# vrgamegirl19/comfyui-vrgamedevgirl

Hardware: NVIDIA H100
Metric: megapixels/sec (grain+LUT+colormatch+sharpen chain) at 4K (higher is better)
Workload: dtype f32

## Files before the change

comfyui-vrgamedevgirl_b200/csrc/vrgdg_kernels.cuh:

```cuda
#pragma once
#include <cuda.h>
#include <cuda_runtime.h>
#include <cuda_fp16.h>
#include <cuda_bf16.h>
#include <stdint.h>
#include "vrgdg_math.cuh"

namespace vrgdg {

enum {
  ST_GRAIN = 1, ST_CM = 2, ST_LUT = 4,
  ST_POST = 8,
  ST_CMF = 16,
  ST_PRE = ST_GRAIN | ST_CM | ST_LUT | ST_CMF
};

template <typename T> struct Elem;
template <> struct Elem<float> {
  static __device__ __forceinline__ float ld(float v) { return v; }
  static __device__ __forceinline__ float st(float v) { return v; }
};
template <> struct Elem<__half> {
  static __device__ __forceinline__ float ld(__half v) { return __half2float(v); }
  static __device__ __forceinline__ __half st(float v) { return __float2half_rn(v); }
};
template <> struct Elem<__nv_bfloat16> {
  static __device__ __forceinline__ float ld(__nv_bfloat16 v) { return __bfloat162float(v); }
  static __device__ __forceinline__ __nv_bfloat16 st(float v) { return __float2bfloat16_rn(v); }
};

template <> struct Elem<uint8_t> {
  static __device__ __forceinline__ float ld(uint8_t v) {
    const float r = 1.0f / 255.0f, f = (float)v, q = __fmul_rn(f, r);
    return __fmaf_rn(__fmaf_rn(-255.0f, q, f), r, q);
  }
  static __device__ __forceinline__ uint8_t st(float v) { return (uint8_t)fminf(fmaxf(mulx(v, 255.0f), 0.0f), 255.0f); }
};

template <typename T> struct Io {
  static constexpr bool BGR = false;
  typedef T noise_t;
  typedef uint4 word_t;
};
template <> struct Io<uint8_t> {
  static constexpr bool BGR = true;
  typedef float noise_t;
  typedef uint32_t word_t;
};
template <typename T> __device__ __forceinline__ float noise_ld(T v) { return Elem<T>::ld(v); }
template <> __device__ __forceinline__ float noise_ld<float>(float v) { return v; }

struct PointParams {
  int B, H, W;
  int64_t hw;
  float gI, gs, goms;
  uint64_t seed;
  int64_t frame0;
  int seed_mode;
  GrainKey gkey;
  const void* ext_noise;
  const float* cm_params;
  float cm_t, cm_omt;
  LutParams lut;
};

#ifndef VRGDG_LUT_POLY
#define VRGDG_LUT_POLY 1
#endif

template <int MASK, bool EXACT>
__device__ __forceinline__ void process_pixel(const PointParams& P, const CmFold& cmf, float zr, float zg, float zb,
                                              float& r, float& g, float& b) {
  if (MASK & ST_GRAIN) {
    if (EXACT) grain_blend_exact(r, g, b, zr, zg, zb, P.gI, P.gs, P.goms);
    else grain_blend_fast(r, g, b, zr, zg, zb, P.gI, P.gs, P.goms);
  }
  if (MASK & ST_CM) {
    colormatch_fold_pixel(r, g, b, cmf);
  }
  if (MASK & ST_CMF) {
    colormatch_from_f(r, g, b, cmf);
  }
  if (MASK & ST_LUT) {
    float x0 = r, x1 = g, x2 = b;
    if (EXACT || !VRGDG_LUT_POLY) lut3d_eval<EXACT>(P.lut, r, g, b);
    else lutp_eval(P.lut, r, g, b);
    if (P.lut.blend < 1.0f) {
      r = lut_blend<EXACT>(x0, r, P.lut.blend, P.lut.one_minus_blend);
      g = lut_blend<EXACT>(x1, g, P.lut.blend, P.lut.one_minus_blend);
      b = lut_blend<EXACT>(x2, b, P.lut.blend, P.lut.one_minus_blend);
    }
  }
}

template <int MASK, bool EXACT>
__device__ __forceinline__ void process_pair(const PointParams& P, const CmFold& cmf, const float* z, float* p) {
  process_pixel<(MASK & ~ST_LUT), EXACT>(P, cmf, z[0], z[1], z[2], p[0], p[1], p[2]);
  process_pixel<(MASK & ~ST_LUT), EXACT>(P, cmf, z[3], z[4], z[5], p[3], p[4], p[5]);
  if (MASK & ST_LUT) {
    float x[6] = {p[0], p[1], p[2], p[3], p[4], p[5]};
    if (EXACT || !VRGDG_LUT_POLY) lut3d_eval2<EXACT>(P.lut, p, p + 3);
    else lutp_eval2(P.lut, p, p + 3);
    if (P.lut.blend < 1.0f) {
#pragma unroll
      for (int i = 0; i < 6; ++i) p[i] = lut_blend<EXACT>(x[i], p[i], P.lut.blend, P.lut.one_minus_blend);
    }
  }
}

template <typename T, int MASK, bool EXACT, bool VEC>
__global__ void __launch_bounds__(256)
k_point(const T* __restrict__ in, T* __restrict__ out, PointParams P,
        int blocks_per_frame, int64_t total_vblocks) {
  typedef typename Io<T>::word_t word_t;
  typedef typename Io<T>::noise_t noise_t;
  constexpr bool BGR = Io<T>::BGR;
  constexpr int PX = VEC ? (int)(3 * sizeof(word_t) / (3 * sizeof(T))) : 1;
  constexpr int NE = PX * 3;
  constexpr bool GRAIN = (MASK & ST_GRAIN) != 0;
  const bool has_ext = GRAIN && (P.ext_noise != nullptr);
  for (int64_t vb = blockIdx.x; vb < total_vblocks; vb += gridDim.x) {
    const int frame = (int)(vb / blocks_per_frame);
    const int bif = (int)(vb - (int64_t)frame * blocks_per_frame);
    const int64_t pix0 = ((int64_t)bif * 256 + threadIdx.x) * PX;
    if (pix0 >= P.hw) continue;
    const int64_t e0 = ((int64_t)frame * P.hw + pix0) * 3;
    const GrainFrame gf = grain_frame(P.seed, P.frame0, frame, P.seed_mode);
    CmFold cmf = {};
    if (MASK & (ST_CM | ST_CMF)) cmf = cm_fold(P.cm_params + (int64_t)frame * 12, P.cm_t, P.cm_omt);
    const uint32_t y = GRAIN ? (uint32_t)pix0 / (uint32_t)P.W : 0u;
    const uint32_t x = GRAIN ? (uint32_t)pix0 - y * (uint32_t)P.W : 0u;

    float v[NE];
    float nz[NE];
    union { word_t q[3]; T e[NE]; } u;
    if (VEC) {
      const word_t* src = reinterpret_cast<const word_t*>(in + e0);
      u.q[0] = __ldg(src); u.q[1] = __ldg(src + 1); u.q[2] = __ldg(src + 2);
    } else {
#pragma unroll
      for (int i = 0; i < NE; ++i) u.e[i] = in[e0 + i];
    }
#pragma unroll
    for (int j = 0; j < PX; ++j) {
#pragma unroll
      for (int c = 0; c < 3; ++c) v[3 * j + c] = Elem<T>::ld(u.e[3 * j + (BGR ? 2 - c : c)]);
    }
    if (has_ext) {
      const noise_t* ns = reinterpret_cast<const noise_t*>(P.ext_noise) + e0;
      if (VEC && sizeof(noise_t) == sizeof(T)) {
        union { word_t q[3]; noise_t e[NE]; } n;
        const word_t* nq = reinterpret_cast<const word_t*>(ns);
        n.q[0] = __ldg(nq); n.q[1] = __ldg(nq + 1); n.q[2] = __ldg(nq + 2);
#pragma unroll
        for (int i = 0; i < NE; ++i) nz[i] = noise_ld<noise_t>(n.e[i]);
      } else {
#pragma unroll
        for (int i = 0; i < NE; ++i) nz[i] = noise_ld<noise_t>(ns[i]);
      }
    }
    if (VEC) {
#pragma unroll
      for (int j = 0; j < PX; j += 2) {
        float z[6] = {0.f, 0.f, 0.f, 0.f, 0.f, 0.f};
        if (GRAIN) {
          if (has_ext) {
#pragma unroll
            for (int i = 0; i < 6; ++i) z[i] = nz[3 * j + i];
          } else {
            grain_pair_normals(grain_pair_bits(P.gkey, gf, (x >> 1) + (uint32_t)(j >> 1), y), z);
          }
        }
        process_pair<MASK, EXACT>(P, cmf, z, &v[3 * j]);
      }
    } else {
      float zr = 0.f, zg = 0.f, zb = 0.f;
      if (GRAIN) {
        if (has_ext) { zr = nz[0]; zg = nz[1]; zb = nz[2]; }
        else grain_pixel_normals(P.gkey, gf, x, y, zr, zg, zb);
      }
      process_pixel<MASK, EXACT>(P, cmf, zr, zg, zb, v[0], v[1], v[2]);
    }
#pragma unroll
    for (int j = 0; j < PX; ++j) {
#pragma unroll
      for (int c = 0; c < 3; ++c) u.e[3 * j + (BGR ? 2 - c : c)] = Elem<T>::st(v[3 * j + c]);
    }
    if (VEC) {
      word_t* dst = reinterpret_cast<word_t*>(out + e0);
      dst[0] = u.q[0]; dst[1] = u.q[1]; dst[2] = u.q[2];
// ... 383 lines not shown
  uint8_t* base = smem_raw + (((smem_a + 127u) & ~127u) - smem_a);
  T* stage0 = reinterpret_cast<T*>(base);
  constexpr bool GPLANE = C::GPLANE;
  float* work = reinterpret_cast<float*>(base + (size_t)NS * C::STAGE_BYTES);
  float* gplane = reinterpret_cast<float*>(base + (size_t)NS * C::STAGE_BYTES + (WORK ? ROWS * BX * 4 : 0));
  uint64_t* bars = reinterpret_cast<uint64_t*>(base + (size_t)NS * C::STAGE_BYTES + (WORK ? ROWS * BX * 4 : 0) + (GPLANE ? ROWS * BX * 4 : 0));

  const int tid = threadIdx.x;
  const uint32_t first = blockIdx.x, stride = gridDim.x, total = (uint32_t)Q.total_tiles;
  const uint32_t n_my = (total > first) ? (total - first + stride - 1) / stride : 0;
  const uint32_t tiles_per_frame = (uint32_t)(Q.tiles_x * Q.tiles_y);
  const bool tma = Q.use_tma != 0;

  if (tma && tid == 0) {
#pragma unroll
    for (int s = 0; s < NS; ++s) mbar_init(&bars[s], 1);
    fence_mbar_init();
    fence_proxy_async();
  }
  __syncthreads();

  auto tile_coords = [&](uint32_t k, int& frame, int& y0, int& x0e) {
    const uint32_t t = first + k * stride;
    const uint32_t f = t / tiles_per_frame;
    const uint32_t rem = t - f * tiles_per_frame;
    const uint32_t ty = rem / (uint32_t)Q.tiles_x;
    frame = (int)f;
    y0 = (int)ty * TY;
    x0e = (int)(rem - ty * (uint32_t)Q.tiles_x) * TXE;
  };
  auto issue = [&](uint32_t k) {
    int frame, y0, x0e;
    tile_coords(k, frame, y0, x0e);
    int s = (int)(k % NS);
    mbar_arrive_expect_tx(&bars[s], (uint32_t)C::STAGE_BYTES);
    tma_load_3d(reinterpret_cast<uint8_t*>(stage0) + (size_t)s * C::STAGE_BYTES, &tmap, x0e - PADL, y0 - 1, frame, &bars[s]);
  };

#ifndef VRGDG_EARLY_REFILL
#define VRGDG_EARLY_REFILL 1
#endif
  constexpr bool EARLY = WORK && (VRGDG_EARLY_REFILL != 0);
  constexpr bool LATE1 = !EARLY && NS == 1;
  constexpr uint32_t AHEAD = EARLY ? NS : (LATE1 ? 1 : NS - 1);
  if (tma && tid == 0) {
    for (uint32_t k = 0; k < AHEAD && k < n_my; ++k) issue(k);
  }

  for (uint32_t k = 0; k < n_my; ++k) {
    int frame, y0, x0e;
    tile_coords(k, frame, y0, x0e);
    const int s = tma ? (int)(k % NS) : 0;
    T* raw = reinterpret_cast<T*>(reinterpret_cast<uint8_t*>(stage0) + (size_t)s * C::STAGE_BYTES);

    if (tma) {
      if (!EARLY && !LATE1 && tid == 0 && k + NS - 1 < n_my) {
        fence_proxy_async();
        issue(k + NS - 1);
      }
      mbar_wait(&bars[s], (uint32_t)((k / NS) & 1));
    } else {
      const T* fbase = in + (int64_t)frame * Q.H * Q.RW;
      for (int i = tid; i < ROWS * BX; i += NT) {
        int r = i / BX, c = i - r * BX;
        int y = y0 - 1 + r, x = x0e - PADL + c;
        T v = Elem<T>::st(0.0f);
        if (y >= 0 && y < Q.H && x >= 0 && x < Q.RW) v = fbase[(int64_t)y * Q.RW + x];
        raw[i] = v;
      }
      __syncthreads();
    }

    if ((MASK & ST_PRE) != 0 || WORK || GPLANE) {
      const PointParams& P = Q.P;
      constexpr bool GRAIN = (MASK & ST_GRAIN) != 0;
      constexpr bool BGR = Io<T>::BGR;
      typedef typename Io<T>::noise_t noise_t;
      const GrainFrame gf = grain_frame(P.seed, P.frame0, frame, P.seed_mode);
      CmFold cmf = {};
      if (MASK & (ST_CM | ST_CMF)) cmf = cm_fold(P.cm_params + (int64_t)frame * 12, P.cm_t, P.cm_omt);
      const bool has_ext = GRAIN && (P.ext_noise != nullptr);
      const GrainFrame pgf = grain_frame(Q.pseed, Q.pframe0, frame, Q.pseed_mode);
      const int pair0 = x0e / 6 - 1;
      for (int i = tid; i < ROWS * C::PAIRS; i += NT) {
        const int r = i / C::PAIRS, kx = i - r * C::PAIRS;
        const int y = y0 - 1 + r, pair = pair0 + kx;
        const int pxa = pair * 2;
        const int so = r * BX + PADL - 6 + 6 * kx;
        const bool rowin = (y >= 0 && y < Q.H);
        const bool need_a = (kx > 0), need_b = (kx < C::PAIRS - 1);
        const bool in_a = need_a && rowin && pxa >= 0 && pxa < Q.W;
        const bool in_b = need_b && rowin && pxa + 1 >= 0 && pxa + 1 < Q.W;
        if (GPLANE) {
          float gz[6] = {0.f, 0.f, 0.f, 0.f, 0.f, 0.f};
          if (rowin && pair >= 0 && pxa < Q.W) {
            float z[6];
            grain_pair_normals(grain_pair_bits(Q.pkey, pgf, (uint32_t)pair, (uint32_t)y), z);
            const float gy0 = Q.poms * z[1], gy1 = Q.poms * z[4];
            const float r0 = fmaf(2.0f * Q.ps, z[0], gy0), g0 = fmaf(Q.ps, z[1], gy0), b0 = fmaf(3.0f * Q.ps, z[2], gy0);
            const float r1 = fmaf(2.0f * Q.ps, z[3], gy1), g1 = fmaf(Q.ps, z[4], gy1), b1 = fmaf(3.0f * Q.ps, z[5], gy1);
            gz[0] = BGR ? b0 : r0; gz[1] = g0; gz[2] = BGR ? r0 : b0;
            gz[3] = BGR ? b1 : r1; gz[4] = g1; gz[5] = BGR ? r1 : b1;
          }
          pair_store6(gplane + so, kx > 0, gz);
        }
        if ((MASK & ST_PRE) == 0 && !WORK) continue;
        float e[6] = {0.f, 0.f, 0.f, 0.f, 0.f, 0.f};
        if (in_a | in_b) {
          pair_load6<T>(raw + so, kx > 0, e);
          float z[6] = {0.f, 0.f, 0.f, 0.f, 0.f, 0.f};
          if (GRAIN) {
            if (has_ext) {
              const noise_t* ns = reinterpret_cast<const noise_t*>(P.ext_noise) + ((int64_t)frame * P.hw + (int64_t)y * Q.W + pxa) * 3;
              if (in_a) { z[0] = noise_ld<noise_t>(ns[0]); z[1] = noise_ld<noise_t>(ns[1]); z[2] = noise_ld<noise_t>(ns[2]); }
              if (in_b) { z[3] = noise_ld<noise_t>(ns[3]); z[4] = noise_ld<noise_t>(ns[4]); z[5] = noise_ld<noise_t>(ns[5]); }
            } else {
              grain_pair_normals(grain_pair_bits(P.gkey, gf, (uint32_t)pair, (uint32_t)y), z);
            }
          }
          float p[6] = {e[BGR ? 2 : 0], e[1], e[BGR ? 0 : 2], e[BGR ? 5 : 3], e[4], e[BGR ? 3 : 5]};
          process_pair<MASK, EXACT>(P, cmf, z, p);
          if (in_a) { e[BGR ? 2 : 0] = p[0]; e[1] = p[1]; e[BGR ? 0 : 2] = p[2]; } else if (WORK) { e[0] = 0.f; e[1] = 0.f; e[2] = 0.f; }
          if (in_b) { e[BGR ? 5 : 3] = p[3]; e[4] = p[4]; e[BGR ? 3 : 5] = p[5]; } else if (WORK) { e[3] = 0.f; e[4] = 0.f; e[5] = 0.f; }
        }
        if constexpr (WORK) {
          pair_store6(work + so, kx > 0, e);
        } else {
          if (in_a | in_b) pair_store6(reinterpret_cast<float*>(raw) + so, kx > 0, e);
        }
      }
      __syncthreads();
      if (EARLY && tma && tid == 0 && k + NS < n_my) {
        fence_proxy_async();
        issue(k + NS);
      }
    }

    if (Q.border == 0) {
      if constexpr (WORK) fix_border<float, C>(work, y0, x0e, Q.H, Q.RW);
      else fix_border<T, C>(raw, y0, x0e, Q.H, Q.RW);
    }

    {
      const float* wt = WORK ? work : nullptr;
      if (Q.exact_stencil) {
        switch (Q.op) {
          case 1: stencil_rows<T, 1, MASK, true>(raw, wt, gplane, out, Q, frame, y0, x0e); break;
          case 2: stencil_rows<T, 2, MASK, true>(raw, wt, gplane, out, Q, frame, y0, x0e); break;
          case 3: stencil_rows<T, 3, MASK, false>(raw, wt, gplane, out, Q, frame, y0, x0e); break;
          case 4: stencil_rows<T, 4, MASK, true>(raw, wt, gplane, out, Q, frame, y0, x0e); break;
          case 5: stencil_rows<T, 5, MASK, false>(raw, wt, gplane, out, Q, frame, y0, x0e); break;
          default: stencil_rows<T, 0, MASK, false>(raw, wt, gplane, out, Q, frame, y0, x0e); break;
        }
      } else {
        switch (Q.op) {
          case 1: stencil_rows<T, 1, MASK, false>(raw, wt, gplane, out, Q, frame, y0, x0e); break;
          case 2: stencil_rows<T, 2, MASK, false>(raw, wt, gplane, out, Q, frame, y0, x0e); break;
          case 3: stencil_rows<T, 3, MASK, false>(raw, wt, gplane, out, Q, frame, y0, x0e); break;
          case 4: stencil_rows<T, 4, MASK, false>(raw, wt, gplane, out, Q, frame, y0, x0e); break;
          case 5: stencil_rows<T, 5, MASK, false>(raw, wt, gplane, out, Q, frame, y0, x0e); break;
          default: stencil_rows<T, 0, MASK, false>(raw, wt, gplane, out, Q, frame, y0, x0e); break;
        }
      }
    }
    if (tma) fence_proxy_async();
    __syncthreads();
    if (LATE1 && tma && tid == 0 && k + 1 < n_my) issue(k + 1);
  }
}

constexpr int MOMENT_BLOCKS = 592;
constexpr int MOMENT_UNIT = 128;

__device__ __forceinline__ double warp_sum(double v) {
#pragma unroll
  for (int o = 16; o > 0; o >>= 1) v += __shfl_xor_sync(0xffffffffu, v, o);
  return v;
}

__device__ __forceinline__ void moments_add(float& r, float& g, float& b, float* s1, float* s2) {
  float fx, fy, fz;
  rgb_to_fxyz(r, g, b, fx, fy, fz);
  r = fx; g = fy; b = fz;
  const float u1 = fx - fy, u2 = fy - fz;
  s1[0] += fy; s1[1] += u1; s1[2] += u2;
  s2[0] = fmaf(fy, fy, s2[0]); s2[1] = fmaf(u1, u1, s2[1]); s2[2] = fmaf(u2, u2, s2[2]);
}

#ifndef VRGDG_MOMENT_SMALL_MINB
#define VRGDG_MOMENT_SMALL_MINB 10
#endif
template <int NT> struct MomentLaunch { static constexpr int MINB = (NT == MOMENT_UNIT) ? VRGDG_MOMENT_SMALL_MINB : 4; };
template <typename T, bool GRAIN, bool VEC, int NT>
__global__ void __launch_bounds__(NT, (MomentLaunch<NT>::MINB))
k_lab_moments(const T* __restrict__ in, PointParams P, int row0, int rows, double* __restrict__ partials, float* __restrict__ fplanes) {
  static_assert(NT % MOMENT_UNIT == 0, "whole reduction units per block");
  constexpr int UPB = NT / MOMENT_UNIT;
  const int unit = blockIdx.x * UPB + (threadIdx.x / MOMENT_UNIT), ut = threadIdx.x % MOMENT_UNIT;
  typedef typename Io<T>::word_t word_t;
  typedef typename Io<T>::noise_t noise_t;
  constexpr bool BGR = Io<T>::BGR;
  constexpr int PX = VEC ? (int)(sizeof(word_t) / sizeof(T)) : 1;
  constexpr int NE = PX * 3;
  const int frame = blockIdx.y;
  const int64_t pbeg = (int64_t)row0 * P.W, n = (int64_t)rows * P.W;
  const T* fbase = in + (int64_t)frame * P.hw * 3;
  const GrainFrame gf = grain_frame(P.seed, P.frame0, frame, P.seed_mode);
  const bool has_ext = GRAIN && (P.ext_noise != nullptr);
  const CmFold nocm = {};
// ... 186 lines not shown
```

comfyui-vrgamedevgirl_b200/csrc/vrgdg_math.cuh:

```cuda
#pragma once
#include <stdint.h>
#include <stddef.h>
#include <string.h>
#include <math.h>

#if defined(__CUDACC__)
#define VRGDG_HD __host__ __device__ __forceinline__
#else
#define VRGDG_HD inline
#endif

namespace vrgdg {

#if defined(__CUDA_ARCH__)
VRGDG_HD float addx(float a, float b) { return __fadd_rn(a, b); }
VRGDG_HD float subx(float a, float b) { return __fsub_rn(a, b); }
VRGDG_HD float mulx(float a, float b) { return __fmul_rn(a, b); }
VRGDG_HD float divx(float a, float b) { return __fdiv_rn(a, b); }
VRGDG_HD float sqrtx(float a) { return __fsqrt_rn(a); }
#else
VRGDG_HD float addx(float a, float b) { volatile float r = a + b; return r; }
VRGDG_HD float subx(float a, float b) { volatile float r = a - b; return r; }
VRGDG_HD float mulx(float a, float b) { volatile float r = a * b; return r; }
VRGDG_HD float divx(float a, float b) { volatile float r = a / b; return r; }
// ... 93 lines not shown
#if defined(__CUDA_ARCH__)
  float l2, rr, sn, cs;
  asm("lg2.approx.ftz.f32 %0, %1;" : "=f"(l2) : "f"(u));
  asm("sqrt.approx.ftz.f32 %0, %1;" : "=f"(rr) : "f"(l2 * -1.3862943611198906f));
  asm("sin.approx.ftz.f32 %0, %1;" : "=f"(sn) : "f"(th));
  asm("cos.approx.ftz.f32 %0, %1;" : "=f"(cs) : "f"(th));
#else
  float rr = sqrtf(-2.0f * logf(u));
  float sn = sinf(th), cs = cosf(th);
#endif
  c = rr * cs;
  s = rr * sn;
}

VRGDG_HD void grain_fields(U4 r, uint32_t* rad, uint32_t* ang) {
  const uint32_t M = 0x1FFFFFu;
  rad[0] = r.x & M;
  ang[0] = ((r.x >> 21) | (r.y << 11)) & M;
  rad[1] = (r.y >> 10) & M;
  ang[1] = r.z & M;
  rad[2] = ((r.z >> 21) | (r.w << 11)) & M;
  ang[2] = (r.w >> 10) & M;
}

VRGDG_HD void grain_pair_normals(U4 r, float* z) {
  uint32_t rad[3], ang[3];
  grain_fields(r, rad, ang);
  float c0, s0, c1, s1, c2, s2;
  box_muller21(rad[0], ang[0], c0, s0);
  box_muller21(rad[1], ang[1], c1, s1);
  box_muller21(rad[2], ang[2], c2, s2);
  z[0] = c0; z[1] = s0; z[2] = c1;
  z[3] = s1; z[4] = c2; z[5] = s2;
}

VRGDG_HD void grain_lane_normals(U4 r, int lane, float& zr, float& zg, float& zb) {
  uint32_t rad[3], ang[3];
  grain_fields(r, rad, ang);
  float c1, s1, ca, sa;
  box_muller21(rad[1], ang[1], c1, s1);
  box_muller21(lane ? rad[2] : rad[0], lane ? ang[2] : ang[0], ca, sa);
  zr = lane ? s1 : ca;
  zg = lane ? ca : sa;
  zb = lane ? sa : c1;
}

VRGDG_HD void grain_pixel_normals(const GrainKey& K, const GrainFrame& f, uint32_t x, uint32_t y, float& zr, float& zg, float& zb) {
  grain_lane_normals(grain_pair_bits(K, f, x >> 1, y), (int)(x & 1u), zr, zg, zb);
}

VRGDG_HD void grain_blend_exact(float& r, float& g, float& b, float zr, float zg, float zb,
                                float I, float s, float oms) {
  float zr2 = mulx(zr, 2.0f);
  float zb3 = mulx(zb, 3.0f);
  float gy = mulx(oms, zg);
  float gr = addx(mulx(s, zr2), gy);
  float gg = addx(mulx(s, zg), gy);
  float gb = addx(mulx(s, zb3), gy);
  r = clamp01(addx(r, mulx(gr, I)));
  g = clamp01(addx(g, mulx(gg, I)));
  b = clamp01(addx(b, mulx(gb, I)));
}

VRGDG_HD void grain_blend_fast(float& r, float& g, float& b, float zr, float zg, float zb,
                               float I, float s, float oms) {
  float gy = oms * zg;
  r = clamp01(fmaf(I, fmaf(2.0f * s, zr, gy), r));
  g = clamp01(fmaf(I, fmaf(s, zg, gy), g));
  b = clamp01(fmaf(I, fmaf(3.0f * s, zb, gy), b));
}

struct LutParams {
  const float* lut;
  const float* lutp;
  int S;
  float smax;
  float dmin[3], dspan[3];
  float blend, one_minus_blend;
  int unit_domain;
};

constexpr int LUT_CELL_FLOATS = 24;

struct F8 { float v[8]; };

VRGDG_HD F8 lut_load8(const float* p) {
  F8 q;
#if defined(__CUDA_ARCH__)
  asm("ld.global.nc.v4.f32 {%0,%1,%2,%3}, [%4];"
      : "=f"(q.v[0]), "=f"(q.v[1]), "=f"(q.v[2]), "=f"(q.v[3]) : "l"(p));
  asm("ld.global.nc.v4.f32 {%0,%1,%2,%3}, [%4+16];"
      : "=f"(q.v[4]), "=f"(q.v[5]), "=f"(q.v[6]), "=f"(q.v[7]) : "l"(p));
#else
  for (int i = 0; i < 8; ++i) q.v[i] = p[i];
#endif
  return q;
}

VRGDG_HD void lut_pack_entry(const float* lut3, int S, int b, int g, int r, float* dst24) {
  const int b1 = (b + 1 < S) ? b + 1 : S - 1, g1 = (g + 1 < S) ? g + 1 : S - 1, r1 = (r + 1 < S) ? r + 1 : S - 1;
  const int cb[8] = {b, b, b, b, b1, b1, b1, b1};
  const int cg[8] = {g, g, g1, g1, g, g, g1, g1};
  const int cr[8] = {r, r1, r, r1, r, r1, r, r1};
#pragma unroll
  for (int k = 0; k < 8; ++k) {
    const float* a = lut3 + ((size_t)(cb[k] * S + cg[k]) * S + cr[k]) * 3;
    dst24[k] = a[0]; dst24[8 + k] = a[1]; dst24[16 + k] = a[2];
  }
}

VRGDG_HD void lut_coord(float v, float dmin, float dspan, bool unit, float smax, int S, int& i0, int& i1, float& f) {
  float n = unit ? v : divx(subx(v, dmin), dspan);
  n = clamp01(n);
  float c = mulx(n, smax);
  float fl = floorf(c);
  i0 = (int)fl;
  i1 = (i0 + 1 < S - 1) ? i0 + 1 : S - 1;
  f = subx(c, fl);
}

template <bool EXACT>
VRGDG_HD float lerp_ref(float a, float b, float f, float omf) {
  if (EXACT) return addx(mulx(a, omf), mulx(b, f));
  return fmaf(f, b - a, a);
}

template <bool EXACT>
VRGDG_HD float lut_channel(const F8& q, float fr, float fg, float fb, float omr, float omg, float omb) {
  const float c00 = lerp_ref<EXACT>(q.v[0], q.v[4], fb, omb);
  const float c01 = lerp_ref<EXACT>(q.v[2], q.v[6], fb, omb);
  const float c10 = lerp_ref<EXACT>(q.v[1], q.v[5], fb, omb);
  const float c11 = lerp_ref<EXACT>(q.v[3], q.v[7], fb, omb);
  const float c0 = lerp_ref<EXACT>(c00, c01, fg, omg);
  const float c1 = lerp_ref<EXACT>(c10, c11, fg, omg);
  return clamp01(lerp_ref<EXACT>(c0, c1, fr, omr));
}

template <bool EXACT>
VRGDG_HD void lut3d_eval(const LutParams& P, float& r, float& g, float& b) {
  int r0, r1, g0, g1, b0, b1;
  float fr, fg, fb;
  lut_coord(r, P.dmin[0], P.dspan[0], P.unit_domain != 0, P.smax, P.S, r0, r1, fr);
  lut_coord(g, P.dmin[1], P.dspan[1], P.unit_domain != 0, P.smax, P.S, g0, g1, fg);
  lut_coord(b, P.dmin[2], P.dspan[2], P.unit_domain != 0, P.smax, P.S, b0, b1, fb);
  (void)r1; (void)g1; (void)b1;
  const float* p = P.lut + (size_t)((b0 * P.S + g0) * P.S + r0) * LUT_CELL_FLOATS;
  const F8 q0 = lut_load8(p), q1 = lut_load8(p + 8), q2 = lut_load8(p + 16);
  const float omb = subx(1.0f, fb), omg = subx(1.0f, fg), omr = subx(1.0f, fr);
  r = lut_channel<EXACT>(q0, fr, fg, fb, omr, omg, omb);
  g = lut_channel<EXACT>(q1, fr, fg, fb, omr, omg, omb);
  b = lut_channel<EXACT>(q2, fr, fg, fb, omr, omg, omb);
}

template <bool EXACT>
VRGDG_HD float lut3d_eval_channel(const LutParams& P, float r, float g, float b, int ch) {
  int r0, r1, g0, g1, b0, b1;
  float fr, fg, fb;
  lut_coord(r, P.dmin[0], P.dspan[0], P.unit_domain != 0, P.smax, P.S, r0, r1, fr);
  lut_coord(g, P.dmin[1], P.dspan[1], P.unit_domain != 0, P.smax, P.S, g0, g1, fg);
  lut_coord(b, P.dmin[2], P.dspan[2], P.unit_domain != 0, P.smax, P.S, b0, b1, fb);
  (void)r1; (void)g1; (void)b1;
  const F8 q = lut_load8(P.lut + (size_t)((b0 * P.S + g0) * P.S + r0) * LUT_CELL_FLOATS + 8 * ch);
  return lut_channel<EXACT>(q, fr, fg, fb, subx(1.0f, fr), subx(1.0f, fg), subx(1.0f, fb));
}

struct LutCell { const float* p; float fr, fg, fb; };

VRGDG_HD LutCell lut_locate(const LutParams& P, float r, float g, float b) {
  int r0, r1, g0, g1, b0, b1;
  LutCell c;
  lut_coord(r, P.dmin[0], P.dspan[0], P.unit_domain != 0, P.smax, P.S, r0, r1, c.fr);
  lut_coord(g, P.dmin[1], P.dspan[1], P.unit_domain != 0, P.smax, P.S, g0, g1, c.fg);
  lut_coord(b, P.dmin[2], P.dspan[2], P.unit_domain != 0, P.smax, P.S, b0, b1, c.fb);
  (void)r1; (void)g1; (void)b1;
  c.p = P.lut + (size_t)((b0 * P.S + g0) * P.S + r0) * LUT_CELL_FLOATS;
  return c;
}

template <bool EXACT>
VRGDG_HD void lut_finish(const LutCell& c, const F8& q0, const F8& q1, const F8& q2, float& r, float& g, float& b) {
  const float omb = subx(1.0f, c.fb), omg = subx(1.0f, c.fg), omr = subx(1.0f, c.fr);
  r = lut_channel<EXACT>(q0, c.fr, c.fg, c.fb, omr, omg, omb);
  g = lut_channel<EXACT>(q1, c.fr, c.fg, c.fb, omr, omg, omb);
  b = lut_channel<EXACT>(q2, c.fr, c.fg, c.fb, omr, omg, omb);
}

template <bool EXACT>
VRGDG_HD void lut3d_eval2(const LutParams& P, float* a, float* b) {
  const LutCell ca = lut_locate(P, a[0], a[1], a[2]), cb = lut_locate(P, b[0], b[1], b[2]);
  const F8 a0 = lut_load8(ca.p), a1 = lut_load8(ca.p + 8), a2 = lut_load8(ca.p + 16);
  const F8 b0 = lut_load8(cb.p), b1 = lut_load8(cb.p + 8), b2 = lut_load8(cb.p + 16);
  lut_finish<EXACT>(ca, a0, a1, a2, a[0], a[1], a[2]);
  lut_finish<EXACT>(cb, b0, b1, b2, b[0], b[1], b[2]);
}

VRGDG_HD void lutp_pack_entry(const float* lut3, int S, int b, int g, int r, float* dst24) {
  float c[LUT_CELL_FLOATS];
  lut_pack_entry(lut3, S, b, g, r, c);
#pragma unroll
  for (int ch = 0; ch < 3; ++ch) {
    double k[8];
#pragma unroll
    for (int i = 0; i < 8; ++i) k[i] = (double)c[8 * ch + i];
#pragma unroll
    for (int bit = 1; bit < 8; bit <<= 1) {
#pragma unroll
      for (int i = 0; i < 8; ++i) if (i & bit) k[i] -= k[i ^ bit];
    }
#pragma unroll
    for (int i = 0; i < 8; ++i) dst24[8 * ch + i] = (float)k[i];
  }
}

VRGDG_HD float lutp_channel(const F8& q, float fr, float fg, float fb) {
  const float a0 = fmaf(fb, q.v[4], q.v[0]), b0 = fmaf(fb, q.v[5], q.v[1]);
  const float a1 = fmaf(fb, q.v[6], q.v[2]), b1 = fmaf(fb, q.v[7], q.v[3]);
  return clamp01(fmaf(fr, fmaf(fg, b1, b0), fmaf(fg, a1, a0)));
}

VRGDG_HD LutCell lutp_locate(const LutParams& P, float r, float g, float b) {
  LutCell c = lut_locate(P, r, g, b);
  c.p = P.lutp + (c.p - P.lut);
  return c;
}
VRGDG_HD void lutp_eval(const LutParams& P, float& r, float& g, float& b) {
  const LutCell c = lutp_locate(P, r, g, b);
  const F8 q0 = lut_load8(c.p), q1 = lut_load8(c.p + 8), q2 = lut_load8(c.p + 16);
  r = lutp_channel(q0, c.fr, c.fg, c.fb); g = lutp_channel(q1, c.fr, c.fg, c.fb); b = lutp_channel(q2, c.fr, c.fg, c.fb);
}
VRGDG_HD void lutp_eval2(const LutParams& P, float* a, float* b) {
  const LutCell ca = lutp_locate(P, a[0], a[1], a[2]), cb = lutp_locate(P, b[0], b[1], b[2]);
  const F8 a0 = lut_load8(ca.p), a1 = lut_load8(ca.p + 8), a2 = lut_load8(ca.p + 16);
  const F8 b0 = lut_load8(cb.p), b1 = lut_load8(cb.p + 8), b2 = lut_load8(cb.p + 16);
  a[0] = lutp_channel(a0, ca.fr, ca.fg, ca.fb); a[1] = lutp_channel(a1, ca.fr, ca.fg, ca.fb); a[2] = lutp_channel(a2, ca.fr, ca.fg, ca.fb);
  b[0] = lutp_channel(b0, cb.fr, cb.fg, cb.fb); b[1] = lutp_channel(b1, cb.fr, cb.fg, cb.fb); b[2] = lutp_channel(b2, cb.fr, cb.fg, cb.fb);
}

template <bool EXACT>
VRGDG_HD float lut_blend(float x, float y, float blend, float omb) {
  if (EXACT) return addx(mulx(x, omb), mulx(y, blend));
  return fmaf(y, blend, x * omb);
}

VRGDG_HD float approx_pow(float x, float e) {
#if defined(__CUDA_ARCH__)
  float l, r;
  asm("lg2.approx.ftz.f32 %0, %1;" : "=f"(l) : "f"(x));
  asm("ex2.approx.ftz.f32 %0, %1;" : "=f"(r) : "f"(l * e));
  return r;
#else
  return exp2f(log2f(x) * e) * (1.0f + 3e-7f);
#endif
}
VRGDG_HD float approx_rcp(float x) {
#if defined(__CUDA_ARCH__)
  float r;
  asm("rcp.approx.ftz.f32 %0, %1;" : "=f"(r) : "f"(x));
  return r;
#else
  return 1.0f / x;
#endif
}
VRGDG_HD float cbrt_pos(float x) {
  const float r = approx_pow(x, -0.33333334f);
  const float r3 = (r * r) * r;
  const float rn = r * fmaf(x * r3, -0.33333334f, 1.3333334f);
  return (x * rn) * rn;
}
VRGDG_HD float inv_root5_pos(float x) {
  const float r = approx_pow(x, -0.2f);
  const float r2 = r * r, r4 = r2 * r2;
  return r * fmaf((x * r) * r4, -0.2f, 1.2f);
}
VRGDG_HD float root5_pos(float x) {
  const float r = inv_root5_pos(x);
  const float r2 = r * r;
  return x * (r2 * r2);
}
VRGDG_HD float pow_2p4(float x) {
  const float s = x * inv_root5_pos(x);
  return (s * s) * s;
}
VRGDG_HD float pow_inv2p4(float x) {
  float y = approx_pow(x, 0.083333336f);
  float y2 = y * y, y4 = y2 * y2, y8 = y4 * y4, y11 = (y8 * y2) * y;
  y = fmaf(fmaf(-y11, y, x), approx_rcp(12.0f * y11), y);
  y2 = y * y;
  return (y2 * y2) * y;
}

VRGDG_HD float srgb_to_linear(float c) {
  const float p = pow_2p4(fmaf(fmaxf(c, 0.04045f), (float)(1.0 / 1.055), (float)(0.055 / 1.055)));
  const float l = c * (float)(1.0 / 12.92);
  return (c > 0.04045f) ? p : l;
}
VRGDG_HD float linear_to_srgb(float l) {
  const float p = fmaf(1.055f, approx_pow(fmaxf(l, 0.0031308f), 0.41666666f), -0.055f);
  const float q = 12.92f * l;
  return (l > 0.0031308f) ? p : q;
}
VRGDG_HD float lab_f(float t) {
  const float p = cbrt_pos(fmaxf(t, 0.008856f));
  const float q = fmaf(7.787f, t, (float)(4.0 / 29.0));
  return (t > 0.008856f) ? p : q;
}
VRGDG_HD void rgb_to_fxyz(float r, float g, float b, float& fx, float& fy, float& fz) {
  const float lr = srgb_to_linear(r), lg = srgb_to_linear(g), lb = srgb_to_linear(b);
  const float x = fmaf((float)(0.180423 / 0.95047), lb, fmaf((float)(0.357580 / 0.95047), lg, (float)(0.412453 / 0.95047) * lr));
  const float y = fmaf(0.072169f, lb, fmaf(0.715160f, lg, 0.212671f * lr));
  const float z = fmaf((float)(0.950227 / 1.08883), lb, fmaf((float)(0.119193 / 1.08883), lg, (float)(0.019334 / 1.08883) * lr));
  fx = lab_f(x); fy = lab_f(y); fz = lab_f(z);
}
VRGDG_HD void rgb_to_lab(float r, float g, float b, float& L, float& A, float& Bv) {
  float fx, fy, fz;
  rgb_to_fxyz(r, g, b, fx, fy, fz);
  L = fmaf(116.0f, fy, -16.0f);
  A = 500.0f * (fx - fy);
  Bv = 200.0f * (fy - fz);
}
// ... 110 lines not shown
```

Baseline: 29030.

## Split 3D LUT cell loads across lane pairs with shuffle exchange

Reorders the packed LUT cell layout so each 4-float half holds one r-slice, then has adjacent lanes share LUT lookups: each lane loads only its half of the cell for both its own and its partner's pixels, computes partial trilinear results, and exchanges them via warp shuffles. The stencil tile loop is made warp-uniform so every lane takes part in the shuffles, with per-lane task guards on the stores. The aim is fewer wide scattered loads per lane and better load coalescing across a lane pair, in exchange for extra shuffle instructions and idle lanes running the LUT path on out-of-range tasks.

Result: faster. 32400, median of 6 (+11.6%).

```diff
diff --git a/comfyui-vrgamedevgirl_b200/csrc/vrgdg_kernels.cuh b/comfyui-vrgamedevgirl_b200/csrc/vrgdg_kernels.cuh
--- a/comfyui-vrgamedevgirl_b200/csrc/vrgdg_kernels.cuh
+++ b/comfyui-vrgamedevgirl_b200/csrc/vrgdg_kernels.cuh
@@ -93,19 +93,24 @@
   }
 }
 
+template <bool EXACT, bool LANE_PAIR>
+__device__ __forceinline__ void lut_pair(const PointParams& P, float* p) {
+  constexpr bool POLY = !EXACT && VRGDG_LUT_POLY;
+  float x[6] = {p[0], p[1], p[2], p[3], p[4], p[5]};
+  if (LANE_PAIR) lut_eval_lane_pair<POLY, EXACT>(P.lut, p, p + 3);
+  else if (POLY) lutp_eval2(P.lut, p, p + 3);
+  else lut3d_eval2<EXACT>(P.lut, p, p + 3);
+  if (P.lut.blend < 1.0f) {
+#pragma unroll
+    for (int i = 0; i < 6; ++i) p[i] = lut_blend<EXACT>(x[i], p[i], P.lut.blend, P.lut.one_minus_blend);
+  }
+}
+
 template <int MASK, bool EXACT>
 __device__ __forceinline__ void process_pair(const PointParams& P, const CmFold& cmf, const float* z, float* p) {
   process_pixel<(MASK & ~ST_LUT), EXACT>(P, cmf, z[0], z[1], z[2], p[0], p[1], p[2]);
   process_pixel<(MASK & ~ST_LUT), EXACT>(P, cmf, z[3], z[4], z[5], p[3], p[4], p[5]);
-  if (MASK & ST_LUT) {
-    float x[6] = {p[0], p[1], p[2], p[3], p[4], p[5]};
-    if (EXACT || !VRGDG_LUT_POLY) lut3d_eval2<EXACT>(P.lut, p, p + 3);
-    else lutp_eval2(P.lut, p, p + 3);
-    if (P.lut.blend < 1.0f) {
-#pragma unroll
-      for (int i = 0; i < 6; ++i) p[i] = lut_blend<EXACT>(x[i], p[i], P.lut.blend, P.lut.one_minus_blend);
-    }
-  }
+  if (MASK & ST_LUT) lut_pair<EXACT, false>(P, p);
 }
 
 template <typename T, int MASK, bool EXACT, bool VEC>
@@ -655,12 +660,15 @@
       const bool has_ext = GRAIN && (P.ext_noise != nullptr);
       const GrainFrame pgf = grain_frame(Q.pseed, Q.pframe0, frame, Q.pseed_mode);
       const int pair0 = x0e / 6 - 1;
-      for (int i = tid; i < ROWS * C::PAIRS; i += NT) {
+      constexpr int TASKS = ROWS * C::PAIRS;
+      for (int i0 = tid & ~31; i0 < TASKS; i0 += NT) {
+        const int i = i0 + (tid & 31);
+        const bool task = i < TASKS;
         const int r = i / C::PAIRS, kx = i - r * C::PAIRS;
         const int y = y0 - 1 + r, pair = pair0 + kx;
         const int pxa = pair * 2;
         const int so = r * BX + PADL - 6 + 6 * kx;
-        const bool rowin = (y >= 0 && y < Q.H);
+        const bool rowin = task && (y >= 0 && y < Q.H);
         const bool need_a = (kx > 0), need_b = (kx < C::PAIRS - 1);
         const bool in_a = need_a && rowin && pxa >= 0 && pxa < Q.W;
         const bool in_b = need_b && rowin && pxa + 1 >= 0 && pxa + 1 < Q.W;
@@ -675,10 +683,11 @@
             gz[0] = BGR ? b0 : r0; gz[1] = g0; gz[2] = BGR ? r0 : b0;
             gz[3] = BGR ? b1 : r1; gz[4] = g1; gz[5] = BGR ? r1 : b1;
           }
-          pair_store6(gplane + so, kx > 0, gz);
+          if (task) pair_store6(gplane + so, kx > 0, gz);
         }
         if ((MASK & ST_PRE) == 0 && !WORK) continue;
         float e[6] = {0.f, 0.f, 0.f, 0.f, 0.f, 0.f};
+        float p[6] = {0.f, 0.f, 0.f, 0.f, 0.f, 0.f};
         if (in_a | in_b) {
           pair_load6<T>(raw + so, kx > 0, e);
           float z[6] = {0.f, 0.f, 0.f, 0.f, 0.f, 0.f};
@@ -691,13 +700,16 @@
               grain_pair_normals(grain_pair_bits(P.gkey, gf, (uint32_t)pair, (uint32_t)y), z);
             }
           }
-          float p[6] = {e[BGR ? 2 : 0], e[1], e[BGR ? 0 : 2], e[BGR ? 5 : 3], e[4], e[BGR ? 3 : 5]};
-          process_pair<MASK, EXACT>(P, cmf, z, p);
+          p[0] = e[BGR ? 2 : 0]; p[1] = e[1]; p[2] = e[BGR ? 0 : 2]; p[3] = e[BGR ? 5 : 3]; p[4] = e[4]; p[5] = e[BGR ? 3 : 5];
+          process_pair<(MASK & ~ST_LUT), EXACT>(P, cmf, z, p);
+        }
+        if (MASK & ST_LUT) lut_pair<EXACT, true>(P, p);
+        if (in_a | in_b) {
           if (in_a) { e[BGR ? 2 : 0] = p[0]; e[1] = p[1]; e[BGR ? 0 : 2] = p[2]; } else if (WORK) { e[0] = 0.f; e[1] = 0.f; e[2] = 0.f; }
           if (in_b) { e[BGR ? 5 : 3] = p[3]; e[4] = p[4]; e[BGR ? 3 : 5] = p[5]; } else if (WORK) { e[3] = 0.f; e[4] = 0.f; e[5] = 0.f; }
         }
         if constexpr (WORK) {
-          pair_store6(work + so, kx > 0, e);
+          if (task) pair_store6(work + so, kx > 0, e);
         } else {
           if (in_a | in_b) pair_store6(reinterpret_cast<float*>(raw) + so, kx > 0, e);
         }
diff --git a/comfyui-vrgamedevgirl_b200/csrc/vrgdg_math.cuh b/comfyui-vrgamedevgirl_b200/csrc/vrgdg_math.cuh
--- a/comfyui-vrgamedevgirl_b200/csrc/vrgdg_math.cuh
+++ b/comfyui-vrgamedevgirl_b200/csrc/vrgdg_math.cuh
@@ -199,26 +199,32 @@
 
 constexpr int LUT_CELL_FLOATS = 24;
 
+struct F4 { float v[4]; };
 struct F8 { float v[8]; };
 
-VRGDG_HD F8 lut_load8(const float* p) {
-  F8 q;
+VRGDG_HD F4 lut_load4(const float* p) {
+  F4 q;
 #if defined(__CUDA_ARCH__)
   asm("ld.global.nc.v4.f32 {%0,%1,%2,%3}, [%4];"
       : "=f"(q.v[0]), "=f"(q.v[1]), "=f"(q.v[2]), "=f"(q.v[3]) : "l"(p));
-  asm("ld.global.nc.v4.f32 {%0,%1,%2,%3}, [%4+16];"
-      : "=f"(q.v[4]), "=f"(q.v[5]), "=f"(q.v[6]), "=f"(q.v[7]) : "l"(p));
-#else
-  for (int i = 0; i < 8; ++i) q.v[i] = p[i];
-#endif
+#else
+  for (int i = 0; i < 4; ++i) q.v[i] = p[i];
+#endif
+  return q;
+}
+
+VRGDG_HD F8 lut_load8(const float* p) {
+  const F4 lo = lut_load4(p), hi = lut_load4(p + 4);
+  F8 q;
+  for (int i = 0; i < 4; ++i) { q.v[i] = lo.v[i]; q.v[4 + i] = hi.v[i]; }
   return q;
 }
 
 VRGDG_HD void lut_pack_entry(const float* lut3, int S, int b, int g, int r, float* dst24) {
   const int b1 = (b + 1 < S) ? b + 1 : S - 1, g1 = (g + 1 < S) ? g + 1 : S - 1, r1 = (r + 1 < S) ? r + 1 : S - 1;
-  const int cb[8] = {b, b, b, b, b1, b1, b1, b1};
+  const int cb[8] = {b, b1, b, b1, b, b1, b, b1};
   const int cg[8] = {g, g, g1, g1, g, g, g1, g1};
-  const int cr[8] = {r, r1, r, r1, r, r1, r, r1};
+  const int cr[8] = {r, r, r, r, r1, r1, r1, r1};
 #pragma unroll
   for (int k = 0; k < 8; ++k) {
     const float* a = lut3 + ((size_t)(cb[k] * S + cg[k]) * S + cr[k]) * 3;
@@ -243,14 +249,17 @@
 }
 
 template <bool EXACT>
+VRGDG_HD float lut_half(const float* h, float fg, float fb, float omg, float omb) {
+  const float cx0 = lerp_ref<EXACT>(h[0], h[1], fb, omb);
+  const float cx1 = lerp_ref<EXACT>(h[2], h[3], fb, omb);
+  return lerp_ref<EXACT>(cx0, cx1, fg, omg);
+}
+template <bool EXACT>
+VRGDG_HD float lut_combine(float c0, float c1, float fr, float omr) { return clamp01(lerp_ref<EXACT>(c0, c1, fr, omr)); }
+
+template <bool EXACT>
 VRGDG_HD float lut_channel(const F8& q, float fr, float fg, float fb, float omr, float omg, float omb) {
-  const float c00 = lerp_ref<EXACT>(q.v[0], q.v[4], fb, omb);
-  const float c01 = lerp_ref<EXACT>(q.v[2], q.v[6], fb, omb);
-  const float c10 = lerp_ref<EXACT>(q.v[1], q.v[5], fb, omb);
-  const float c11 = lerp_ref<EXACT>(q.v[3], q.v[7], fb, omb);
-  const float c0 = lerp_ref<EXACT>(c00, c01, fg, omg);
-  const float c1 = lerp_ref<EXACT>(c10, c11, fg, omg);
-  return clamp01(lerp_ref<EXACT>(c0, c1, fr, omr));
+  return lut_combine<EXACT>(lut_half<EXACT>(q.v, fg, fb, omg, omb), lut_half<EXACT>(q.v + 4, fg, fb, omg, omb), fr, omr);
 }
 
 template <bool EXACT>
@@ -283,14 +292,18 @@
 
 struct LutCell { const float* p; float fr, fg, fb; };
 
+VRGDG_HD int lut_cell_offset(const LutParams& P, float r, float g, float b, float& fr, float& fg, float& fb) {
+  int r0, r1, g0, g1, b0, b1;
+  lut_coord(r, P.dmin[0], P.dspan[0], P.unit_domain != 0, P.smax, P.S, r0, r1, fr);
+  lut_coord(g, P.dmin[1], P.dspan[1], P.unit_domain != 0, P.smax, P.S, g0, g1, fg);
+  lut_coord(b, P.dmin[2], P.dspan[2], P.unit_domain != 0, P.smax, P.S, b0, b1, fb);
+  (void)r1; (void)g1; (void)b1;
+  return ((b0 * P.S + g0) * P.S + r0) * LUT_CELL_FLOATS;
+}
+
 VRGDG_HD LutCell lut_locate(const LutParams& P, float r, float g, float b) {
-  int r0, r1, g0, g1, b0, b1;
   LutCell c;
-  lut_coord(r, P.dmin[0], P.dspan[0], P.unit_domain != 0, P.smax, P.S, r0, r1, c.fr);
-  lut_coord(g, P.dmin[1], P.dspan[1], P.unit_domain != 0, P.smax, P.S, g0, g1, c.fg);
-  lut_coord(b, P.dmin[2], P.dspan[2], P.unit_domain != 0, P.smax, P.S, b0, b1, c.fb);
-  (void)r1; (void)g1; (void)b1;
-  c.p = P.lut + (size_t)((b0 * P.S + g0) * P.S + r0) * LUT_CELL_FLOATS;
+  c.p = P.lut + lut_cell_offset(P, r, g, b, c.fr, c.fg, c.fb);
   return c;
 }
 
@@ -320,7 +333,7 @@
 #pragma unroll
     for (int i = 0; i < 8; ++i) k[i] = (double)c[8 * ch + i];
 #pragma unroll
-    for (int bit = 1; bit < 8; bit <<= 1) {
+    for (int bit = 4; bit >= 1; bit >>= 1) {
 #pragma unroll
       for (int i = 0; i < 8; ++i) if (i & bit) k[i] -= k[i ^ bit];
     }
@@ -329,10 +342,11 @@
   }
 }
 
+VRGDG_HD float lutp_half(const float* h, float fg, float fb) { return fmaf(fg, fmaf(fb, h[3], h[2]), fmaf(fb, h[1], h[0])); }
+VRGDG_HD float lutp_combine(float a, float b, float fr) { return clamp01(fmaf(fr, b, a)); }
+
 VRGDG_HD float lutp_channel(const F8& q, float fr, float fg, float fb) {
-  const float a0 = fmaf(fb, q.v[4], q.v[0]), b0 = fmaf(fb, q.v[5], q.v[1]);
-  const float a1 = fmaf(fb, q.v[6], q.v[2]), b1 = fmaf(fb, q.v[7], q.v[3]);
-  return clamp01(fmaf(fr, fmaf(fg, b1, b0), fmaf(fg, a1, a0)));
+  return lutp_combine(lutp_half(q.v, fg, fb), lutp_half(q.v + 4, fg, fb), fr);
 }
 
 VRGDG_HD LutCell lutp_locate(const LutParams& P, float r, float g, float b) {
@@ -352,6 +366,52 @@
   a[0] = lutp_channel(a0, ca.fr, ca.fg, ca.fb); a[1] = lutp_channel(a1, ca.fr, ca.fg, ca.fb); a[2] = lutp_channel(a2, ca.fr, ca.fg, ca.fb);
   b[0] = lutp_channel(b0, cb.fr, cb.fg, cb.fb); b[1] = lutp_channel(b1, cb.fr, cb.fg, cb.fb); b[2] = lutp_channel(b2, cb.fr, cb.fg, cb.fb);
 }
+
+#if defined(__CUDACC__)
+template <bool POLY, bool EXACT>
+__device__ __forceinline__ void lut_eval_lane_pair(const LutParams& P, float* a, float* b) {
+  const unsigned FULL = 0xffffffffu;
+  const bool odd = (threadIdx.x & 1) != 0;
+  float fr[2], fg[2], fb[2];
+  int cell[2];
+  cell[0] = lut_cell_offset(P, a[0], a[1], a[2], fr[0], fg[0], fb[0]);
+  cell[1] = lut_cell_offset(P, b[0], b[1], b[2], fr[1], fg[1], fb[1]);
+  int qc[4];
+  float qg[4], qb[4];
+#pragma unroll
+  for (int k = 0; k < 2; ++k) {
+    const int pc = __shfl_xor_sync(FULL, cell[k], 1);
+    const float pg = __shfl_xor_sync(FULL, fg[k], 1), pb = __shfl_xor_sync(FULL, fb[k], 1);
+    qc[k] = odd ? pc : cell[k];     qg[k] = odd ? pg : fg[k];     qb[k] = odd ? pb : fb[k];
+    qc[2 + k] = odd ? cell[k] : pc; qg[2 + k] = odd ? fg[k] : pg; qb[2 + k] = odd ? fb[k] : pb;
+  }
+  const float* tab = (POLY ? P.lutp : P.lut) + (odd ? 4 : 0);
+  F4 q[4][3];
+#pragma unroll
+  for (int k = 0; k < 4; ++k)
+#pragma unroll
+    for (int ch = 0; ch < 3; ++ch) q[k][ch] = lut_load4(tab + qc[k] + 8 * ch);
+  float h[4][3];
+#pragma unroll
+  for (int k = 0; k < 4; ++k) {
+    const float omg = subx(1.0f, qg[k]), omb = subx(1.0f, qb[k]);
+#pragma unroll
+    for (int ch = 0; ch < 3; ++ch) h[k][ch] = POLY ? lutp_half(q[k][ch].v, qg[k], qb[k]) : lut_half<EXACT>(q[k][ch].v, qg[k], qb[k], omg, omb);
+  }
+  float* px[2] = {a, b};
+#pragma unroll
+  for (int k = 0; k < 2; ++k) {
+    const float omr = subx(1.0f, fr[k]);
+#pragma unroll
+    for (int ch = 0; ch < 3; ++ch) {
+      const float mine = odd ? h[2 + k][ch] : h[k][ch];
+      const float other = __shfl_xor_sync(FULL, odd ? h[k][ch] : h[2 + k][ch], 1);
+      const float c0 = odd ? other : mine, c1 = odd ? mine : other;
+      px[k][ch] = POLY ? lutp_combine(c0, c1, fr[k]) : lut_combine<EXACT>(c0, c1, fr[k], omr);
+    }
+  }
+}
+#endif
 
 template <bool EXACT>
 VRGDG_HD float lut_blend(float x, float y, float blend, float omb) {
```
